# XiYe20/NPVP

Measured on AMD Instinct MI355X. Metric: predictor train frames/sec, higher is better.
Workload: dtype f32 (two-term fp16 split of amax-scaled operands, 3 MFMAs per product, fp32 accumulate: fp32-grade; small GEMMs: three-term bf16 split)

## Files before the change

include/npvp_hip.h:

```cpp
#ifndef NPVP_HIP_H
#define NPVP_HIP_H
#include <stddef.h>
#ifdef __cplusplus
extern "C" {
#endif

typedef struct ihipStream_t* npvp_stream_t;

int npvp_version(void);
const char* npvp_last_error(void);
long long npvp_launch_count(void);
void* npvp_stream_create_low_priority(int* least, int* greatest);
int npvp_stream_destroy(void* stream);
void* npvp_event_create(void);
int npvp_event_record(void* event, void* stream);
float npvp_event_elapsed_ms(void* event0, void* event1);
int npvp_event_destroy(void* event);

long long npvp_graph_node_counts(void* graph, long long* counts, long long* memset_bytes, int max_memsets);

long long npvp_gemm_workspace_bytes(int M, int N, int K);
int npvp_gemm_kernel_id(int a_kc, int b_kc, int M, int N, int K, int precision, int has_planes);
int npvp_gemm_route(int a_kc, int b_kc, int M, int N, int K, int precision, int has_planes, int plain_epilogue, int* out4);
int npvp_gemm_f32(int a_kc, int b_kc, int M, int N, int K, const float* A, long long lda, const float* B, long long ldb,
// ... 15 lines not shown
                              int frames, float eps, npvp_stream_t stream);
int npvp_split_weight(const float* w, long long ld, int N, int K, void* F, void* D, npvp_stream_t stream);
int npvp_split_weights_batched(const void* desc, int count, npvp_stream_t stream);
int npvp_amax(const float* x, long long rows, long long cols, long long ld, float* slot, npvp_stream_t stream);

typedef struct npvp_reduce_job {
  const float* ws; float* out; long long ldc; int M, N, splits, accum; float alpha; int blocks; const float* cs_part; float* cs_out;
} npvp_reduce_job_t;
int npvp_wgrad_f16_chainable(int M, int N, int K);
long long npvp_wgrad_f16_chain_workspace_bytes(int M, int N, int K);
int npvp_wgrad_f16_chained(int M, int N, int K, const float* dy, long long lda, const float* x, long long ldb, float* dw,
                           long long ldc, float* db, int accumulate, const float* a_amax, const float* b_amax,
                           unsigned int* range_flag, float adrop_p, int adrop_g1, int adrop_g2, unsigned int adrop_salt,
                           const unsigned long long* seed, const void* prev_job, void* my_job, void* workspace,
                           long long ws_bytes, npvp_stream_t stream);
int npvp_splitk_reduce_job(const void* job, npvp_stream_t stream);
int npvp_splitk_reduce_multi(const void* jobs, int n, npvp_stream_t stream);
int npvp_linear_bwd_f16_takes(int R, int N, int K);
int npvp_linear_bwd_f16(int R, int N, int K, const float* dy, long long ldy, const float* dy_amax, const void* w_planes_d,
                        const float* w_amax, float* dx, long long ldx, int act, const float* aux_in, const float* residual,
                        long long ldr, float drop_p, int drop_mode, int drop_g1, int drop_g2, unsigned int drop_salt, float* dx_amax,
                        const float* x, long long ldxx, const float* x_amax, float* dw, long long ldw, float* db,
                        unsigned int* range_flag, float adrop_p, int adrop_g1, int adrop_g2, unsigned int adrop_salt,
                        const unsigned long long* seed, const void* prev_job, void* my_job, void* workspace, long long ws_bytes,
                        npvp_stream_t stream);
int npvp_linear_bwd_f16_skip(int R, int N, int K, const float* dy, long long ldy, const float* dy_amax, const void* w_planes_d,
                             const float* w_amax, float* dx, long long ldx, int act, const float* aux_in, const float* residual,
                             long long ldr, float drop_p, int drop_mode, int drop_g1, int drop_g2, unsigned int drop_salt,
                             float* dx_amax, const float* x, long long ldxx, const float* x_amax, float* dw, long long ldw, float* db,
                             unsigned int* range_flag, float adrop_p, int adrop_g1, int adrop_g2, unsigned int adrop_salt,
// ... 220 lines not shown
```

npvp_amd/csrc/gemm.h:

```cpp
#pragma once
#include <type_traits>
#include "common.h"

namespace npvp {

typedef float f32x16 __attribute__((ext_vector_type(16)));
typedef __bf16 bf16x8 __attribute__((ext_vector_type(8)));
typedef __bf16 bf16x4 __attribute__((ext_vector_type(4)));

struct ReduceJob {
  const float* ws; float* out; long long ldc; int M, N, splits, accum; float alpha; int blocks; const float* cs_part; float* cs_out;
};

struct GemmParams {
  const float* A; const float* B; float* C;
  const float* bias;
  const float* residual;
  float* aux_out;
  const float* aux_in;
  float* rowstats;
  float* colsum;
  const unsigned long long* seed;
  long long lda, ldb, ldc, ldr;
  int M, N, K;
// ... 269 lines not shown

inline int wgrad_splits(int M, int N, int K, int min_rows) {
  if ((K & 15) || M < 64 || N < 128 || K < min_rows) return 0;
  const int tiles = ((M + 127) / 128) * ((N + 255) / 256);
  int s = (512 + tiles - 1) / tiles;
  const int maxs = K / 256;
  if (s > maxs) s = maxs;
  if (s > 64) s = 64;
  if (s >= 8) s &= ~7;
  while (s > 1 && (K % (s * 16)) != 0) --s;
  return s < 1 ? 1 : s;
}
inline int wide_wgrad_splits(int M, int N, int K) { return wgrad_splits(M, N, K, 32768); }
inline int f16_wgrad_splits(int M, int N, int K) { return wgrad_splits(M, N, K, 1024); }

inline bool adrop_args_ok(float p, int g1, int g2, const unsigned long long* seed, bool rows16) {
  return p >= 0.f && p < 0.5f && (p == 0.f || (seed && g1 > 0 && g2 > 0 && (!rows16 || g1 % 16 == 0)));
}

int wide_variant(int M, int N, int K);
void launch_gemm_wide(GemmParams& p, int variant, hipStream_t stream);
void launch_gemm_wgrad_wide(GemmParams& p, hipStream_t stream);
int gemm_f16_variant(int M, int N, int K);
void launch_gemm_f16(GemmParams& p, int variant, hipStream_t stream);
void launch_gemm_wgrad_f16(GemmParams& p, hipStream_t stream);

}
```

npvp_amd/csrc/gemm.hip:

```cpp
#include "gemm.h"
#include "partials.h"
#include <type_traits>

namespace npvp {

constexpr int BM = 128, BN = 128, BK = 32, GEMM_THREADS = 256;

template <bool KC> struct Stager;

template <> struct Stager<true> {
  static constexpr int LD = 129;
  float4 r[4];
  __device__ __forceinline__ void load(const float* src, long long ld, int row0, int nrows, int k0) {
    const int t = threadIdx.x;
    const int kc = (t & 7) * 4;
#pragma unroll
    for (int i = 0; i < 4; ++i) {
      const int row = row0 + (t >> 3) + 32 * i;
      r[i] = (row < nrows) ? ld4(src + (long long)row * ld + k0 + kc) : make_float4(0.f, 0.f, 0.f, 0.f);
    }
  }
  __device__ __forceinline__ void store(float* s) const {
    const int t = threadIdx.x;
    const int kc = (t & 7) * 4;
// ... 490 lines not shown
              p.accum, cs_here ? (const float*)p.colsum : nullptr, cs_here ? colsum_a : nullptr, p.c_amax);
  NPVP_CHECK_LAUNCH();
  if (!colsum_a || cs_here) return NPVP_OK;
  return finish_partials(make_partials(p.colsum, 0, p.splits, p.splits, p.M, colsum_a, p.accum).job, 0, stream, "gemm: column-sum reduce launch failed");
}

extern "C" int npvp_gemm_f32_skip(int a_kc, int b_kc, int M, int N, int K, const float* A, long long lda, const float* B,
                                  long long ldb, float* C, long long ldc, const float* bias, int act, const float* aux_in,
                                  float* aux_out, const float* residual, long long ldr, float drop_p, int drop_mode,
                                  int drop_g1, int drop_g2, const unsigned long long* seed, unsigned int salt, float alpha,
                                  int precision, float* colsum_a, const void* b_pre, int accumulate, float* rowstats,
                                  const float* a_amax, const float* b_amax, float* c_amax, unsigned int* range_flag,
                                  float adrop_p, int adrop_g1, int adrop_g2, unsigned int adrop_salt,
                                  float skip_p, int skip_g1, int skip_g2, unsigned int skip_salt,
                                  void* workspace, long long ws_bytes, hipStream_t stream) {
  NPVP_CHECK_ARG(skip_p >= 0.f && skip_p < 1.f && (skip_p == 0.f || (seed && skip_g1 > 0 && skip_g2 > 0 && a_kc)),
                 "gemm: the row skip needs a device seed, row groups and a row-major A");
  NPVP_CHECK_ARG(M > 0 && N > 0 && K > 0, "gemm: empty problem");
  NPVP_CHECK_ARG(precision == 0 || precision == 4 || precision == 5 || precision == 6,
                 "gemm: precision must be 0 (exact fp32-input MFMA), 4 (three-term bf16 split, 6 MFMAs per product: "
                 "fp32-grade), 5 (two-term bf16 split, 3 MFMAs per product, ~2^-16) or 6 (two-term fp16 split with amax-scaled "
                 "operands, 3 MFMAs per product: fp32-grade; shapes it does not take run as 4)");
  const bool want_h = precision == 6;
  NPVP_CHECK_ARG(K % BK == 0, "gemm: K must be a multiple of 32");
  NPVP_CHECK_ARG(M % 4 == 0 && N % 4 == 0, "gemm: M and N must be multiples of 4");
  NPVP_CHECK_ARG(((uintptr_t)A % 16) == 0 && ((uintptr_t)B % 16) == 0 && ((uintptr_t)C % 16) == 0, "gemm: pointers must be 16-byte aligned");
  NPVP_CHECK_ARG(lda % 4 == 0 && ldb % 4 == 0, "gemm: lda/ldb must be multiples of 4 floats");
  NPVP_CHECK_ARG(ldc % 4 == 0 && (!residual || (ldr % 4 == 0 && ((uintptr_t)residual % 16) == 0)) && (!bias || ((uintptr_t)bias % 16) == 0) &&
                 (!aux_in || ((uintptr_t)aux_in % 16) == 0) && (!aux_out || ((uintptr_t)aux_out % 16) == 0),
                 "gemm: ldc / ldr must be multiples of 4 floats and bias / aux / residual 16-byte aligned (float4 epilogue)");
  NPVP_CHECK_ARG(!(a_kc == 0 && b_kc == 1), "gemm: (a_kc=0,b_kc=1) is not used by the path");
  NPVP_CHECK_ARG((act != 3 && act != 4) || aux_in, "gemm: act 3/4 need aux_in");
// ... 75 lines not shown
```

npvp_amd/csrc/gemm_f16.hip:

```cpp
#include "gemm.h"
#include <cstdio>
#include <cstdlib>

namespace npvp {

typedef _Float16 f16x8 __attribute__((ext_vector_type(8)));
typedef _Float16 f16x4 __attribute__((ext_vector_type(4)));
typedef __attribute__((address_space(1))) const void* gptr_t;
typedef __attribute__((address_space(3))) void* lptr_t;
typedef float f32x4 __attribute__((ext_vector_type(4)));

__device__ __forceinline__ void split_f16_scaled(const f32x4 v, const float s, f16x4& hi, f16x4& lo) {
  unsigned int h01, h23, l01, l23;
  asm("v_fma_mixlo_f16 %0, %1, %2, 0" : "=v"(h01) : "v"(v[0]), "v"(s));
  asm("v_fma_mixlo_f16 %0, %1, %2, 0" : "=v"(h23) : "v"(v[2]), "v"(s));
  asm("v_fma_mixhi_f16 %0, %1, %2, 0" : "+v"(h01) : "v"(v[1]), "v"(s));
  asm("v_fma_mixhi_f16 %0, %1, %2, 0" : "+v"(h23) : "v"(v[3]), "v"(s));
  asm("v_fma_mixlo_f16 %0, %1, %2, -%3 op_sel_hi:[0,0,1]" : "=v"(l01) : "v"(v[0]), "v"(s), "v"(h01));
  asm("v_fma_mixlo_f16 %0, %1, %2, -%3 op_sel_hi:[0,0,1]" : "=v"(l23) : "v"(v[2]), "v"(s), "v"(h23));
  asm("v_fma_mixhi_f16 %0, %1, %2, -%3 op_sel:[0,0,1] op_sel_hi:[0,0,1]" : "+v"(l01) : "v"(v[1]), "v"(s), "v"(h01));
  asm("v_fma_mixhi_f16 %0, %1, %2, -%3 op_sel:[0,0,1] op_sel_hi:[0,0,1]" : "+v"(l23) : "v"(v[3]), "v"(s), "v"(h23));
  typedef unsigned int u32x2 __attribute__((ext_vector_type(2)));
  const u32x2 hp = {h01, h23}, lp = {l01, l23};
  hi = __builtin_bit_cast(f16x4, hp);
// ... 301 lines not shown
    float cm = 0.f;
    splitk_reduce_body(p.prev, (by - p.splits) * gx + bx, p.prev.blocks, cm);
    return;
  }
  int z, tl;
  {
    const int tiles = gx;
    if (p.splits > 1 && (p.splits & 7) == 0) {
      const int lin = bx + tiles * by, xcd = lin & 7, slot = lin >> 3;
      const int g = slot / tiles;
      tl = slot - g * tiles; z = g * 8 + xcd;
    } else { z = by; tl = bx; }
  }
  const int tile_m = tl / p.tiles_n, tile_n = tl - tile_m * p.tiles_n;
  const int m0 = tile_m * BM, n0 = tile_n * BN;
  const float* A = p.A + (long long)z * p.K * p.lda;
  const float* B = p.B + (long long)z * p.K * p.ldb;
  const int t = threadIdx.x, lane = t & 63, wave = __builtin_amdgcn_readfirstlane(t >> 6);
  const int wm = wave / WN, wn = wave % WN, r = lane & 31, h = lane >> 5;
  const int nk = p.K >> 4;
  const float sa = amax_scale(amax_slot_read(p.a_amax)), sb = amax_scale(amax_slot_read(p.b_amax));

  f32x16 acc[TM][TN];
#pragma unroll
  for (int i = 0; i < TM; ++i)
#pragma unroll
    for (int j = 0; j < TN; ++j)
#pragma unroll
      for (int g = 0; g < 16; ++g) acc[i][j][g] = 0.f;

  const int ka = t >> 5, cqa = t & 31, kb = t >> 6, cqb = t & 63;
  const char* a_base = reinterpret_cast<const char*>(A);
  const char* b_base = reinterpret_cast<const char*>(B);
  const unsigned int a_voff = (unsigned int)(((long long)ka * p.lda + min(m0 + 4 * cqa, p.M - 4)) * 4);
  const unsigned int b_voff = (unsigned int)(((long long)kb * p.ldb + min(n0 + 4 * cqb, p.N - 4)) * 4);
  const long long a_row8 = 32 * p.lda, b_row4 = 16 * p.ldb, a_step = 64 * p.lda, b_step = 64 * p.ldb;
  const int a_dst = ka * ROWA + ((8 * cqa) ^ ((ka & 3) << 6));
  const int b_dst = A_BYTES + kb * ROWB + ((8 * cqb) ^ ((kb & 3) << 6));
  const int q = (lane >> 2) & 3, pp = lane & 3, cg = 16 * ((lane >> 4) & 1) + 4 * pp;
  int fa[TM], fb[TN];
#pragma unroll
  for (int i = 0; i < TM; ++i) fa[i] = (8 * h + q) * ROWA + (((wm * TM * 32 + i * 32 + cg) * 2) ^ (q << 6));
#pragma unroll
  for (int j = 0; j < TN; ++j) fb[j] = A_BYTES + (8 * h + q) * ROWB + (((wn * TN * 32 + j * 32 + cg) * 2) ^ (q << 6));

  const bool want_cs = p.colsum && tile_n == 0;
  f32x4 cs = {0.f, 0.f, 0.f, 0.f};
  f32x4 cm4 = {0.f, 0.f, 0.f, 0.f};
  f32x4 ra[2], rb[4];
#define NPVP_G_LOAD(KT)                                                                                     \
  { const int kt_ = min((KT), nk - 1);                                                                      \
    const char* pa_ = a_base + (long long)kt_ * a_step; const char* pb_ = b_base + (long long)kt_ * b_step;  \
    asm volatile("global_load_dwordx4 %0, %1, %2" : "=v"(ra[0]) : "v"(a_voff), "s"(pa_) : "memory");        \
    asm volatile("global_load_dwordx4 %0, %1, %2" : "=v"(ra[1]) : "v"(a_voff), "s"(pa_ + a_row8) : "memory"); \
    _Pragma("unroll") for (int i_ = 0; i_ < 4; ++i_)                                                        \
      asm volatile("global_load_dwordx4 %0, %1, %2" : "=v"(rb[i_]) : "v"(b_voff), "s"(pb_ + i_ * b_row4) : "memory"); }
#define NPVP_G_WAIT(N, ...) asm volatile("s_waitcnt vmcnt(" #N ")" : __VA_ARGS__ :: "memory");
#define NPVP_G_STORE(DST, V, SC, PLANE)                                                                     \
  { f16x4 hi_, lo_; split_f16_scaled((V), (SC), hi_, lo_);                                                  \
    *reinterpret_cast<f16x4*>(DST) = hi_; *reinterpret_cast<f16x4*>((DST) + (PLANE)) = lo_; }
  const unsigned long long aseed = p.adrop.thresh ? *p.seed : 0ull;
  const long long arow0 = (long long)z * p.K;
  float am_ = 1.f;
#define NPVP_G_AMASK(KT) { if (p.adrop.thresh) am_ = drop_spec_scale(p.adrop, aseed, arow0 + 16ll * min((KT), nk - 1), 0, 1); }
#define NPVP_G_STORE_A(ST) { const float sam_ = sa * am_;                                                                        \
    if (p.range_flag) cm4 = __builtin_elementwise_max(cm4, __builtin_elementwise_max(__builtin_elementwise_abs(ra[0]), __builtin_elementwise_abs(ra[1]))); \
    NPVP_G_STORE((ST) + a_dst, ra[0], sam_, A_PLANE) NPVP_G_STORE((ST) + a_dst + 8 * ROWA, ra[1], sam_, A_PLANE) }
#define NPVP_G_STORE_B(ST, I) NPVP_G_STORE((ST) + b_dst + (I) * 4 * ROWB, rb[I], sb, B_PLANE)

  NPVP_G_LOAD(0)
  NPVP_G_AMASK(0)
  NPVP_G_WAIT(0, "+v"(ra[0]), "+v"(ra[1]), "+v"(rb[0]), "+v"(rb[1]), "+v"(rb[2]), "+v"(rb[3]))
  if (want_cs) cs += (ra[0] + ra[1]) * am_;
  NPVP_G_STORE_A(lds)
  NPVP_G_STORE_B(lds, 0) NPVP_G_STORE_B(lds, 1) NPVP_G_STORE_B(lds, 2) NPVP_G_STORE_B(lds, 3)
  NPVP_G_LOAD(1)
  __syncthreads();

#define NPVP_G_STEP(KT, CUR, NXT)                                                                            \
  {                                                                                                          \
    const char* st_ = lds + (CUR) * STAGE;                                                                   \
    char* nx_ = lds + (NXT) * STAGE;                                                                         \
    NPVP_G_WAIT(3, "+v"(ra[0]), "+v"(ra[1]), "+v"(rb[0]))                                                    \
    NPVP_G_AMASK((KT) + 1)                                                         \
    if (want_cs && (KT) + 1 < nk) { asm volatile("" ::: "memory"); cs += (ra[0] + ra[1]) * am_; }   \
    f16x8 fa_[TM][2];                                                                                        \
    _Pragma("unroll") for (int i_ = 0; i_ < TM; ++i_)                                                        \
      _Pragma("unroll") for (int s_ = 0; s_ < 2; ++s_) fa_[i_][s_] = lds_read_tr_pair_h(st_ + fa[i_] + s_ * A_PLANE, 4 * ROWA); \
// ... 9 lines not shown
    }                                                                                                        \
     \
    __builtin_amdgcn_sched_barrier(0);                                                                       \
    asm volatile("s_waitcnt lgkmcnt(0)" ::: "memory");                                                       \
    __builtin_amdgcn_s_barrier();                                                                            \
  }

  int kt = 0;
  for (; kt + 1 < nk; kt += 2) {
    NPVP_G_STEP(kt, 0, 1)
    NPVP_G_STEP(kt + 1, 1, 0)
  }
  if (kt < nk) NPVP_G_STEP(kt, 0, 1)
  asm volatile("s_waitcnt vmcnt(0)" : "+v"(ra[0]), "+v"(ra[1]), "+v"(rb[0]), "+v"(rb[1]), "+v"(rb[2]), "+v"(rb[3]) :: "memory");
  if (p.range_flag) {
    float* red = reinterpret_cast<float*>(lds);
    *reinterpret_cast<f32x4*>(red + ka * BM + 4 * cqa) = cm4;
    __syncthreads();
    bool flag = false;
    if (t < BM) {
      float m = red[t];
#pragma unroll
      for (int i = 1; i < 8; ++i) m = fmaxf(m, red[i * BM + t]);
      const int et = (int)((__float_as_uint(sa) >> 23) & 0xffu), e = (int)((__float_as_uint(m) >> 23) & 0xffu);
      const int d = 268 - et - e;
      flag = e >= 16 && e != 255 && d >= 18 && m0 + t < p.M;
    }
    const bool any = __builtin_amdgcn_ballot_w64(flag) != 0ull;
    if (any && lane == 0) atomicAdd(p.range_flag, 1u);
    __syncthreads();
// ... 68 lines not shown
  long long want = (total4 + 255) / 256;
  if (want > 256) want = 256;
  if (want < 1) want = 1;
  return (int)((want + tiles - 1) / tiles);
}

static dim3 size_gemm_wgrad_f16(GemmParams& p) {
  p.tiles_m = (p.M + 127) / 128;
  p.tiles_n = (p.N + 255) / 256;
  const int tiles = p.tiles_m * p.tiles_n, rr = reduce_rows_for(p.prev, tiles);
  p.prev.blocks = rr * tiles;
  return dim3(tiles, p.splits + rr);
}

void launch_gemm_wgrad_f16(GemmParams& p, hipStream_t stream) {
  const dim3 grid = size_gemm_wgrad_f16(p);
  NPVP_LAUNCH((gemm_wgrad_f16_kernel<2, 4, 2, 2>), grid, dim3(256), 0, stream, p);
}

static bool deferred_wgrad_args_ok(const char* who, const float* dy, long long lda, const float* x, long long ldb, const float* dw, long long ldc, float adrop_p,
                                   int adrop_g1, int adrop_g2, const unsigned long long* seed, const void* workspace, long long ws_bytes, long long ws_need) {
  const char* what = ((((uintptr_t)dy | (uintptr_t)x | (uintptr_t)dw) & 15) || ((lda | ldb | ldc) & 3)) ? "operands must be 16-byte aligned with leading dimensions that are multiples of 4"
                     : !adrop_args_ok(adrop_p, adrop_g1, adrop_g2, seed, true) ? "adrop needs a device seed and groups of a multiple of 16 rows"
                     : (!workspace || ws_bytes < ws_need) ? "workspace too small" : nullptr;
  char msg[192];
  if (what) { snprintf(msg, sizeof(msg), "%s: %s", who, what); npvp_set_error(msg); }
  return !what;
}

static GemmParams deferred_wgrad_params(int M, int N, int K, const float* dy, long long lda, const float* x, long long ldb, const float* a_amax, const float* b_amax,
// ... 157 lines not shown
  NPVP_CHECK_LAUNCH();
  return NPVP_OK;
}

static_assert(sizeof(ReduceJob) == sizeof(npvp_reduce_job_t), "npvp_reduce_job_t (include/npvp_hip.h) mirrors this layout");

extern "C" int npvp_wgrad_f16_chainable(int M, int N, int K) {
  return (M % 4 == 0 && N % 4 == 0 && f16_wgrad_splits(M, N, K) > 1) ? 1 : 0;
}

extern "C" long long npvp_wgrad_f16_chain_workspace_bytes(int M, int N, int K) {
  const int s = f16_wgrad_splits(M, N, K);
  return s > 1 ? splitk_workspace_bytes(s, M, N) : 0;
}

extern "C" int npvp_wgrad_f16_chained(int M, int N, int K, const float* dy, long long lda, const float* x, long long ldb, float* dw,
                                      long long ldc, float* db, int accumulate, const float* a_amax, const float* b_amax,
                                      unsigned int* range_flag, float adrop_p, int adrop_g1, int adrop_g2, unsigned int adrop_salt,
                                      const unsigned long long* seed, const void* prev_job, void* my_job, void* workspace,
                                      long long ws_bytes, hipStream_t stream) {
  NPVP_CHECK_ARG(npvp_wgrad_f16_chainable(M, N, K), "wgrad_f16_chained: shape not taken (npvp_wgrad_f16_chainable tells)");
  NPVP_CHECK_ARG(dy && x && dw && a_amax && b_amax && my_job, "wgrad_f16_chained: null operand / amax slot / job");
  if (!deferred_wgrad_args_ok("wgrad_f16_chained", dy, lda, x, ldb, dw, ldc, adrop_p, adrop_g1, adrop_g2, seed, workspace, ws_bytes,
                              npvp_wgrad_f16_chain_workspace_bytes(M, N, K))) return NPVP_ERR_ARG;
  NPVP_CHECK_ARG(!db || ((uintptr_t)db % 16) == 0, "wgrad_f16_chained: the bias gradient must be 16-byte aligned");
  GemmParams p = deferred_wgrad_params(M, N, K, dy, lda, x, ldb, a_amax, b_amax, range_flag, make_drop_spec(adrop_p, adrop_salt, 1, adrop_g1, adrop_g2),
                                       seed, prev_job, workspace, db != nullptr, accumulate);
  launch_gemm_wgrad_f16(p, stream);
  NPVP_CHECK_LAUNCH();
  leave_reduce_job(p, dw, ldc, db, my_job);
  return NPVP_OK;
}

extern "C" int npvp_linear_bwd_f16_takes(int R, int N, int K) {
  const int v = gemm_f16_variant(R, K, N);
  return ((v == 2 || v == 3 || v == 4) && npvp_wgrad_f16_chainable(N, K, R)) ? 1 : 0;
}

extern "C" int npvp_linear_bwd_f16_skip(int R, int N, int K, const float* dy, long long ldy, const float* dy_amax, const void* w_planes_d,
                                        const float* w_amax, float* dx, long long ldx, int act, const float* aux_in, const float* residual,
                                        long long ldr, float drop_p, int drop_mode, int drop_g1, int drop_g2, unsigned int drop_salt,
                                        float* dx_amax, const float* x, long long ldxx, const float* x_amax, float* dw, long long ldw, float* db,
                                        unsigned int* range_flag, float adrop_p, int adrop_g1, int adrop_g2, unsigned int adrop_salt,
                                        float skip_p, int skip_g1, int skip_g2, unsigned int skip_salt,
                                        const unsigned long long* seed, const void* prev_job, void* my_job, void* workspace,
                                        long long ws_bytes, hipStream_t stream) {
// ... 98 lines not shown
```

npvp_amd/ops.py:

```python
import functools
import os
from collections import namedtuple

import torch

from ._lib import lib, check
from . import sched as _S
from .sched import (_p, _ptr, _stream, _ws, AmaxSlot, GemmProbe, HbmProbe, ProbeEvent, AuxStream, StepContext, current, use, scoped,
                    remember, rng, GradSink, WgradStream, WgradChain, ReduceQueue, RangeGuard)


def amax_of(t, slot=None):
    if slot is not None:
        return slot
    for cand in (t, t._base):
        tag = getattr(cand, "_npvp_amax", None) if cand is not None else None
        if tag is not None and tag[1] == cand._version:
            return tag[0]
    s = AmaxSlot.new(t.device)
    t2 = t if t.dim() == 2 else t.reshape(-1, t.shape[-1])
    if t2.stride(1) != 1:
        t2 = t2.contiguous()
    check(lib().npvp_amax(_ptr(t2), t2.shape[0], t2.shape[1], t2.stride(0), _ptr(s), _stream()), "npvp_amax")
    t._npvp_amax = (s, t._version)
# ... 358 lines not shown

def masked_grad(dy2, drop, w):
    if not drop.on:
        return dy2, NO_DROP
    R, N = dy2.shape
    K = w.shape[1]
    if (drop.mode == 1 and drop.g1 % 16 == 0 and drop.p < 0.5 and GEMM_PRECISION == 6 and R <= DROP_PATH_IN_GEMM_ROWS
            and _planes(w, "D", R) is not None and _gemm_kernel_id(1, 0, R, K, N, 6, True) in (5, 7) and _h16(N, K, R, 6)):
        return dy2, drop
    return drop_apply(dy2, drop), NO_DROP


DROP_PATH_IN_GEMM_ROWS = 1 << 30


def linear_wgrad(dy, x, with_bias_grad=False, into=None, into_b=None, dy_amax=None, x_amax=None, a_drop=NO_DROP):
    R, N = dy.shape
    K = x.shape[1]
    acc = into is not None
    dw = into if acc else torch.empty(N, K, dtype=torch.float32, device=dy.device)
    db = (into_b if acc else torch.empty(N, dtype=torch.float32, device=dy.device)) if with_bias_grad else None
    c = _S._cur
    g = c.range_guard
    plan = wgrad_plan(N, K, R, GEMM_PRECISION, WGRAD_PRECISION, acc, a_drop.on, g.fallback, g.strict, c.wgrad.in_flush, c.wgrad.enabled,
                      c.grad_sink.listener is not None, c.chain.enabled, dy.stride(1) == 1 and x.stride(1) == 1 and dw.stride(1) == 1)
    flag = g.flag(dy.device) if plan.watch else None
    if plan.route == "strict":
        tw = torch.empty(N, K, dtype=torch.float32, device=dy.device)
        tb = torch.empty(N, dtype=torch.float32, device=dy.device) if with_bias_grad else None
        gemm(0, 0, N, K, R, dy, dy.stride(0), x, x.stride(0), tw, colsum_a=tb, a_amax=dy_amax, b_amax=x_amax, range_flag=flag)
        if g.poll(dy.device):
            g.fallback = False
            gemm(0, 0, N, K, R, dy, dy.stride(0), x, x.stride(0), tw, colsum_a=tb, precision=4)
        if acc:
            dw.add_(tw)
            if tb is not None:
                db.add_(tb)
        else:
            dw, db = tw, tb
    elif plan.route == "chained":
        c.chain.launch(dy, x, dw, db, amax_of(dy, dy_amax), amax_of(x, x_amax), a_drop, flag)
    else:
        gemm(0, 0, N, K, R, dy, dy.stride(0), x, x.stride(0), dw, colsum_a=db, accumulate=acc, precision=plan.precision, a_amax=dy_amax,
             b_amax=x_amax, a_drop=a_drop, range_flag=flag)
    return (dw, db) if with_bias_grad else dw


class FusedLinearBwd:
    enabled = True
    MAX_ROWS = 16384
    with_gradient_stream = False

    @classmethod
    def takes(cls, R, N, K):
        return linear_bwd_plan(R, N, K, 6, True, False, True, True, True, True, False, cls.MAX_ROWS).fused


def linear_bwd(dy, x, w, b, sk, act=0, aux_in=None, drop=NO_DROP, residual=None, dy_amax=None, dx_amax=None, a_drop=NO_DROP,
               row_skip=NO_DROP):
    R, N = dy.shape
    K = w.shape[1]
    has_b = b is not None
    c = _S._cur
    sunk = _sunk(sk, has_b)
    pl = _planes(w, "D", R)
    plan = linear_bwd_plan(R, N, K, GEMM_PRECISION, sunk, c.wgrad.enabled, not (c.range_guard.fallback or c.range_guard.strict),
                           dy.stride(1) == 1 and x.stride(1) == 1 and (not sunk or sk[0][0].stride(1) == 1), pl is not None,
                           FusedLinearBwd.enabled, FusedLinearBwd.with_gradient_stream, FusedLinearBwd.MAX_ROWS)
    if not plan.fused:
        dx = linear_dgrad(dy, w, act=act, aux_in=aux_in, drop=drop, residual=residual, dy_amax=dy_amax, dx_amax=dx_amax, a_drop=a_drop,
                          row_skip=row_skip)
        gw, gb = _lin_grads(dy, x, w, b, sk, a_drop=a_drop, plan=plan)
        return dx, gw, gb
    planes, w_amax = pl
    gw, gb = sk[0][0], (sk[1][0] if has_b else None)
    dev = dy.device
    dy_amax, x_amax = amax_of(dy, dy_amax), amax_of(x)
    dx = torch.empty(R, K, dtype=torch.float32, device=dev)
    ws, wsn = _ws(c.chain.workspace_bytes(N, K, R), dev)
    st = _stream()
    seed = c.rng.seed_tensor(dev) if (drop.on or a_drop.on or row_skip.on) else None
    outs = (gw.data_ptr(),) if gb is None else (gw.data_ptr(), gb.data_ptr())
    later = c.chain if plan.reduction == "chained" else c.reduce
    job_addr, prev_addr = later.job_slot(st, outs)
    pe = GemmProbe.begin(8)
    head = (R, N, K, dy.data_ptr(), dy.stride(0), dy_amax.data_ptr(), planes.data_ptr(), w_amax.data_ptr(), dx.data_ptr(), dx.stride(0),
            act, _ptr(aux_in), _ptr(residual), 0 if residual is None else residual.stride(0), drop.p, drop.mode, drop.g1, drop.g2,
# ... 418 lines not shown
        if ctx.needs_input_grad[0] and ctx.needs_input_grad[1]:
            dz, ad = masked_grad(dy2, ctx.drop, w)
        else:
            dz, ad = (drop_apply(dy2, ctx.drop) if ctx.drop.on else dy2), NO_DROP
        dx = linear_dgrad(dz, w, a_drop=ad).reshape(ctx.xshape) if ctx.needs_input_grad[0] else None
        dw = db = None
        want_b = ctx.has_b and ctx.needs_input_grad[2]
        if ctx.needs_input_grad[1]:
            dw, db = _lin_grads(dz, x2, w, True if want_b else None, ctx.sink, a_drop=ad)
        elif want_b:
            db = colsum(dz)
        dres = dy if ctx.has_r else None
        return dx, dw, db, dres, None, None


def _lin_grads(dy, x, w, b, sk, a_drop=NO_DROP, plan=None):
    has_b = b is not None
    if plan is None:
        plan = linear_bwd_plan(dy.shape[0], dy.shape[1], x.shape[1], GEMM_PRECISION, _sunk(sk, has_b), _S._cur.wgrad.enabled)
    if not plan.sunk:
        g = linear_wgrad(dy, x, has_b, a_drop=a_drop)
        return (g[0], g[1]) if has_b else (g, None)
    a1, a2 = (amax_of(dy), amax_of(x)) if plan.fill_slots else (None, None)
    fn = lambda dy=dy, x=x, gw=sk[0][0], gb=(sk[1][0] if has_b else None), a1=a1, a2=a2, ad=a_drop: \
        linear_wgrad(dy, x, has_b, into=gw, into_b=gb, dy_amax=a1, x_amax=a2, a_drop=ad)
    if plan.on_grad_stream:
        _S._cur.wgrad.run(fn, dy, x, wrote=sk, urgent=plan.urgent)
    else:
        fn()
        _S._cur.grad_sink.wrote(*sk)
    return None, None


def _wb_sink(w, b):
    sw = _S._cur.grad_sink.slot(w)
    if sw is None:
        return None
    if b is None or not b.requires_grad:
        return (sw, None)
    sb = _S._cur.grad_sink.slot(b)
# ... 450 lines not shown
            gdww = gdwb = None
        else:
            gdww = torch.empty(hid, 1, 3, 3, dtype=torch.float32, device=dev)
            check(L.npvp_transpose(_ptr(dwtb), _ptr(gdww), 1, 9, hid, _stream()), "npvp_transpose")
            gdwb = dwtb[9]
        dh1, gn1w, gn1b = _fln_bwd(da1, h1, stats[0], stats[1], n1w, n1b, frames, 64 * hid, NO_DROP, NO_DROP, 1, s_n1,
                                      psum=psum, nparts=nparts, skip=skip)
        del da1
        dx, gw1, gb1 = linear_bwd(dh1, x, w1, True if has_b1 else None, s_fc1, row_skip=rs)
        return (dx, dout if has_res else None, gw1, gb1, gn1w, gn1b, gdww, gdwb, gn2w, gn2b, gw2, gb2, gn3w, gn3b,
                None, None, None, None)


MID_BWD_N2 = True
DROP_PATH_SKIP = True


def mlpdwbn_fused_supported(R, C, hid, Co, H, W):
    return (GEMM_PRECISION in (4, 6) and H == 8 and W == 8 and R % 64 == 0 and hid % 512 == 0 and Co % 128 == 0 and hid % 128 == 0
            and C % 32 == 0)


def mlpdwbn(x, res, w1, b1, n1w, n1b, dww, dwb, n2w, n2b, w2, b2, n3w, n3b, frames, T, p_drop, p_dp):
    return _MlpDwbn.apply(x, res, w1, b1, n1w, n1b, dww, dwb, n2w, n2b, w2, b2, n3w, n3b, frames, T, p_drop, p_dp)


def _raw_ln_fwd(x2, w, b, eps, relu=0):
    rows, C = x2.shape
    y = torch.empty_like(x2)
    st = torch.empty(2, rows, dtype=torch.float32, device=x2.device)
# ... 658 lines not shown
```

npvp_amd/sched.py:

```python
import contextlib
import ctypes
import functools
import os

import torch

from ._lib import lib, check

_p = ctypes.c_void_p


def _ptr(t):
    return None if t is None else t.data_ptr()


_raw_stream = getattr(torch._C, "_cuda_getCurrentRawStream", None)
_cur_dev = getattr(torch._C, "_cuda_getDevice", None) or torch.cuda.current_device


def _stream():
    if _raw_stream is not None:
        return _raw_stream(_cur_dev())
    return torch.cuda.current_stream().cuda_stream

# ... 447 lines not shown

    def job_added(self, st, out_ptrs, keep, wrote):
        job, prev = self._open
        if prev is not None and prev[2] is not None:
            self.ctx.grad_sink.wrote(*prev[2])
        self._pending[st] = (job, keep, wrote)
        if not self.ctx.wgrad.in_flush:
            self.ctx.reduce.arm()

    def launch(self, dy, x, dw, db, dy_amax, x_amax, a_drop, flag):
        R, N = dy.shape
        K = x.shape[1]
        st = _stream()
        ws, wsn = _ws(self.workspace_bytes(N, K, R), dy.device)
        job_addr, prev_addr = self.job_slot(st)
        seed = self.ctx.rng.seed_tensor(dy.device) if a_drop.on else None
        pe = GemmProbe.begin(6)
        check(lib().npvp_wgrad_f16_chained(N, K, R, _ptr(dy), dy.stride(0), _ptr(x), x.stride(0), _ptr(dw), dw.stride(0), _ptr(db), 1,
                                           _ptr(dy_amax), _ptr(x_amax), _ptr(flag), a_drop.p, a_drop.g1, a_drop.g2, a_drop.salt,
                                           _ptr(seed), prev_addr, job_addr, _ptr(ws), wsn, st), "npvp_wgrad_f16_chained")
        GemmProbe.end(pe, 2.0 * N * K * R, 4.0 * (N * R + K * R + N * K), (0, 0), 6)
        self.job_added(st, None, (ws, dw, db), None)

    def flush(self):
        st = _stream()
        prev = self._pending.pop(st, None)
        if prev is not None:
            check(lib().npvp_splitk_reduce_job(ctypes.addressof(prev[0]), st), "npvp_splitk_reduce_job")
            if prev[2] is not None:
                self.ctx.grad_sink.wrote(*prev[2])


class RangeGuardState:
    mode = os.environ.get("NPVP_RANGE_GUARD", "on")
    strict = mode == "strict"
# ... 146 lines not shown
```

Before: 8443.

## Skip dropped drop-path row groups in the chained fp16 weight-gradient GEMM

The split-K fp16 weight-gradient kernel now builds, per block, a compacted list of row groups (K-dimension instances) kept by the drop-path mask. It then iterates only over their K steps, redistributing the remaining steps evenly across splits. The mask is evaluated with a ballot and prefix count in shared memory. Python routes the row-skip spec into the chained and generic wgrad paths. This avoids loading and multiplying rows whose gradient is zero because the whole sample path was dropped. The cost is extra per-block setup, a readfirstlane-indexed address walk, and handling of splits that end up empty.

```diff
diff --git a/include/npvp_hip.h b/include/npvp_hip.h
--- a/include/npvp_hip.h
+++ b/include/npvp_hip.h
@@ -53,6 +53,11 @@
                            unsigned int* range_flag, float adrop_p, int adrop_g1, int adrop_g2, unsigned int adrop_salt,
                            const unsigned long long* seed, const void* prev_job, void* my_job, void* workspace,
                            long long ws_bytes, npvp_stream_t stream);
+int npvp_wgrad_f16_chained_skip(int M, int N, int K, const float* dy, long long lda, const float* x, long long ldb, float* dw,
+                                long long ldc, float* db, int accumulate, const float* a_amax, const float* b_amax,
+                                unsigned int* range_flag, float adrop_p, int adrop_g1, int adrop_g2, unsigned int adrop_salt,
+                                float skip_p, int skip_g1, int skip_g2, unsigned int skip_salt, const unsigned long long* seed,
+                                const void* prev_job, void* my_job, void* workspace, long long ws_bytes, npvp_stream_t stream);
 int npvp_splitk_reduce_job(const void* job, npvp_stream_t stream);
 int npvp_splitk_reduce_multi(const void* jobs, int n, npvp_stream_t stream);
 int npvp_linear_bwd_f16_takes(int R, int N, int K);
diff --git a/npvp_amd/csrc/gemm.h b/npvp_amd/csrc/gemm.h
--- a/npvp_amd/csrc/gemm.h
+++ b/npvp_amd/csrc/gemm.h
@@ -307,6 +307,16 @@
 inline int wide_wgrad_splits(int M, int N, int K) { return wgrad_splits(M, N, K, 32768); }
 inline int f16_wgrad_splits(int M, int N, int K) { return wgrad_splits(M, N, K, 1024); }
 
+constexpr int KSKIP_MAX_INSTANCES = 256;
+__host__ __device__ inline int kskip_real_step(const unsigned short* kept, int S, int j) { return (int)kept[j / S] * S + j % S; }
+__host__ __device__ inline void kskip_split_range(int nkk, int splits, int z, int& j0, int& j1) {
+  const long long q = ((long long)nkk + splits - 1) / splits, a = q * z, b = a + q;
+  j0 = (int)(a < nkk ? a : nkk); j1 = (int)(b < nkk ? b : nkk);
+}
+inline bool kskip_takes(long long rows, int g1) {
+  return g1 > 0 && g1 % 16 == 0 && rows % g1 == 0 && rows / g1 <= KSKIP_MAX_INSTANCES;
+}
+
 inline bool adrop_args_ok(float p, int g1, int g2, const unsigned long long* seed, bool rows16) {
   return p >= 0.f && p < 0.5f && (p == 0.f || (seed && g1 > 0 && g2 > 0 && (!rows16 || g1 % 16 == 0)));
 }
diff --git a/npvp_amd/csrc/gemm.hip b/npvp_amd/csrc/gemm.hip
--- a/npvp_amd/csrc/gemm.hip
+++ b/npvp_amd/csrc/gemm.hip
@@ -528,8 +528,8 @@
                                   float adrop_p, int adrop_g1, int adrop_g2, unsigned int adrop_salt,
                                   float skip_p, int skip_g1, int skip_g2, unsigned int skip_salt,
                                   void* workspace, long long ws_bytes, hipStream_t stream) {
-  NPVP_CHECK_ARG(skip_p >= 0.f && skip_p < 1.f && (skip_p == 0.f || (seed && skip_g1 > 0 && skip_g2 > 0 && a_kc)),
-                 "gemm: the row skip needs a device seed, row groups and a row-major A");
+  NPVP_CHECK_ARG(skip_p >= 0.f && skip_p < 1.f && (skip_p == 0.f || (seed && skip_g1 > 0 && skip_g2 > 0 && (a_kc || !b_kc))),
+                 "gemm: the row skip needs a device seed, row groups and a row-major A or a weight-gradient layout");
   NPVP_CHECK_ARG(M > 0 && N > 0 && K > 0, "gemm: empty problem");
   NPVP_CHECK_ARG(precision == 0 || precision == 4 || precision == 5 || precision == 6,
                  "gemm: precision must be 0 (exact fp32-input MFMA), 4 (three-term bf16 split, 6 MFMAs per product: "
diff --git a/npvp_amd/csrc/gemm_f16.hip b/npvp_amd/csrc/gemm_f16.hip
--- a/npvp_amd/csrc/gemm_f16.hip
+++ b/npvp_amd/csrc/gemm_f16.hip
@@ -339,11 +339,34 @@
   }
   const int tile_m = tl / p.tiles_n, tile_n = tl - tile_m * p.tiles_n;
   const int m0 = tile_m * BM, n0 = tile_n * BN;
-  const float* A = p.A + (long long)z * p.K * p.lda;
-  const float* B = p.B + (long long)z * p.K * p.ldb;
   const int t = threadIdx.x, lane = t & 63, wave = __builtin_amdgcn_readfirstlane(t >> 6);
   const int wm = wave / WN, wn = wave % WN, r = lane & 31, h = lane >> 5;
-  const int nk = p.K >> 4;
+  __shared__ unsigned short kept_inst[KSKIP_MAX_INSTANCES];
+  __shared__ int kept_wave[NW];
+  int nk = p.K >> 4, kstep0 = z * nk;
+  int S = 0x7fffffff, wstep = 0, winst = 0;
+  if (p.rskip.thresh) {
+    const int I = (int)((long long)p.K * p.splits / p.rskip.g1);
+    const unsigned int grp = (unsigned int)t - div_by_magic((unsigned int)t, p.rskip.m2, p.rskip.s2) * (unsigned int)p.rskip.g2;
+    const bool keep = t < I && rng_u32(*p.seed, p.rskip.salt, (uint64_t)grp) >= p.rskip.thresh;
+    const unsigned long long bal = __builtin_amdgcn_ballot_w64(keep);
+    if (lane == 0) kept_wave[wave] = __builtin_popcountll(bal);
+    __syncthreads();
+    int before = 0, kept = 0;
+#pragma unroll
+    for (int w = 0; w < NW; ++w) { const int c = kept_wave[w]; before += w < wave ? c : 0; kept += c; }
+    if (keep) kept_inst[before + __builtin_popcountll(bal & ((1ull << lane) - 1ull))] = (unsigned short)t;
+    __syncthreads();
+    kept = __builtin_amdgcn_readfirstlane(kept);
+    S = p.rskip.g1 >> 4;
+    int j0, j1;
+    kskip_split_range(S * kept, p.splits, z, j0, j1);
+    nk = j1 - j0; kstep0 = 0;
+    if (nk > 0) {
+      winst = j0 / S; wstep = j0 - winst * S;
+      kstep0 = __builtin_amdgcn_readfirstlane((int)kept_inst[winst]) * S + wstep;
+    }
+  }
   const float sa = amax_scale(amax_slot_read(p.a_amax)), sb = amax_scale(amax_slot_read(p.b_amax));
 
   f32x16 acc[TM][TN];
@@ -355,8 +378,8 @@
       for (int g = 0; g < 16; ++g) acc[i][j][g] = 0.f;
 
   const int ka = t >> 5, cqa = t & 31, kb = t >> 6, cqb = t & 63;
-  const char* a_base = reinterpret_cast<const char*>(A);
-  const char* b_base = reinterpret_cast<const char*>(B);
+  const char* a_base = reinterpret_cast<const char*>(p.A);
+  const char* b_base = reinterpret_cast<const char*>(p.B);
   const unsigned int a_voff = (unsigned int)(((long long)ka * p.lda + min(m0 + 4 * cqa, p.M - 4)) * 4);
   const unsigned int b_voff = (unsigned int)(((long long)kb * p.ldb + min(n0 + 4 * cqb, p.N - 4)) * 4);
   const long long a_row8 = 32 * p.lda, b_row4 = 16 * p.ldb, a_step = 64 * p.lda, b_step = 64 * p.ldb;
@@ -373,9 +396,13 @@
   f32x4 cs = {0.f, 0.f, 0.f, 0.f};
   f32x4 cm4 = {0.f, 0.f, 0.f, 0.f};
   f32x4 ra[2], rb[4];
+  int kld = kstep0;
 #define NPVP_G_LOAD(KT)                                                                                     \
-  { const int kt_ = min((KT), nk - 1);                                                                      \
-    const char* pa_ = a_base + (long long)kt_ * a_step; const char* pb_ = b_base + (long long)kt_ * b_step;  \
+  { if ((KT) > 0 && (KT) < nk) {                                                                            \
+      ++kld;                                                                                                \
+      if (++wstep == S) { wstep = 0; ++winst; kld = __builtin_amdgcn_readfirstlane((int)kept_inst[winst]) * S; } \
+    }                                                                                                       \
+    const char* pa_ = a_base + (long long)kld * a_step; const char* pb_ = b_base + (long long)kld * b_step;  \
     asm volatile("global_load_dwordx4 %0, %1, %2" : "=v"(ra[0]) : "v"(a_voff), "s"(pa_) : "memory");        \
     asm volatile("global_load_dwordx4 %0, %1, %2" : "=v"(ra[1]) : "v"(a_voff), "s"(pa_ + a_row8) : "memory"); \
     _Pragma("unroll") for (int i_ = 0; i_ < 4; ++i_)                                                        \
@@ -385,9 +412,8 @@
   { f16x4 hi_, lo_; split_f16_scaled((V), (SC), hi_, lo_);                                                  \
     *reinterpret_cast<f16x4*>(DST) = hi_; *reinterpret_cast<f16x4*>((DST) + (PLANE)) = lo_; }
   const unsigned long long aseed = p.adrop.thresh ? *p.seed : 0ull;
-  const long long arow0 = (long long)z * p.K;
   float am_ = 1.f;
-#define NPVP_G_AMASK(KT) { if (p.adrop.thresh) am_ = drop_spec_scale(p.adrop, aseed, arow0 + 16ll * min((KT), nk - 1), 0, 1); }
+#define NPVP_G_AMASK(KT) { if (p.adrop.thresh) am_ = drop_spec_scale(p.adrop, aseed, 16ll * kld, 0, 1); }
 #define NPVP_G_STORE_A(ST) { const float sam_ = sa * am_;                                                                        \
     if (p.range_flag) cm4 = __builtin_elementwise_max(cm4, __builtin_elementwise_max(__builtin_elementwise_abs(ra[0]), __builtin_elementwise_abs(ra[1]))); \
     NPVP_G_STORE((ST) + a_dst, ra[0], sam_, A_PLANE) NPVP_G_STORE((ST) + a_dst + 8 * ROWA, ra[1], sam_, A_PLANE) }
@@ -396,7 +422,7 @@
   NPVP_G_LOAD(0)
   NPVP_G_AMASK(0)
   NPVP_G_WAIT(0, "+v"(ra[0]), "+v"(ra[1]), "+v"(rb[0]), "+v"(rb[1]), "+v"(rb[2]), "+v"(rb[3]))
-  if (want_cs) cs += (ra[0] + ra[1]) * am_;
+  if (want_cs && nk > 0) cs += (ra[0] + ra[1]) * am_;
   NPVP_G_STORE_A(lds)
   NPVP_G_STORE_B(lds, 0) NPVP_G_STORE_B(lds, 1) NPVP_G_STORE_B(lds, 2) NPVP_G_STORE_B(lds, 3)
   NPVP_G_LOAD(1)
@@ -436,6 +462,7 @@
   if (kt < nk) NPVP_G_STEP(kt, 0, 1)
   asm volatile("s_waitcnt vmcnt(0)" : "+v"(ra[0]), "+v"(ra[1]), "+v"(rb[0]), "+v"(rb[1]), "+v"(rb[2]), "+v"(rb[3]) :: "memory");
   if (p.range_flag) {
+    if (nk == 0) cm4 = f32x4{0.f, 0.f, 0.f, 0.f};
     float* red = reinterpret_cast<float*>(lds);
     *reinterpret_cast<f32x4*>(red + ka * BM + 4 * cqa) = cm4;
     __syncthreads();
@@ -534,6 +561,7 @@
 }
 
 void launch_gemm_wgrad_f16(GemmParams& p, hipStream_t stream) {
+  if (p.rskip.thresh && !(p.seed && kskip_takes((long long)p.K * p.splits, p.rskip.g1))) p.rskip.thresh = 0u;
   const dim3 grid = size_gemm_wgrad_f16(p);
   NPVP_LAUNCH((gemm_wgrad_f16_kernel<2, 4, 2, 2>), grid, dim3(256), 0, stream, p);
 }
@@ -721,11 +749,14 @@
   return s > 1 ? splitk_workspace_bytes(s, M, N) : 0;
 }
 
-extern "C" int npvp_wgrad_f16_chained(int M, int N, int K, const float* dy, long long lda, const float* x, long long ldb, float* dw,
-                                      long long ldc, float* db, int accumulate, const float* a_amax, const float* b_amax,
-                                      unsigned int* range_flag, float adrop_p, int adrop_g1, int adrop_g2, unsigned int adrop_salt,
-                                      const unsigned long long* seed, const void* prev_job, void* my_job, void* workspace,
-                                      long long ws_bytes, hipStream_t stream) {
+extern "C" int npvp_wgrad_f16_chained_skip(int M, int N, int K, const float* dy, long long lda, const float* x, long long ldb, float* dw,
+                                           long long ldc, float* db, int accumulate, const float* a_amax, const float* b_amax,
+                                           unsigned int* range_flag, float adrop_p, int adrop_g1, int adrop_g2, unsigned int adrop_salt,
+                                           float skip_p, int skip_g1, int skip_g2, unsigned int skip_salt,
+                                           const unsigned long long* seed, const void* prev_job, void* my_job, void* workspace,
+                                           long long ws_bytes, hipStream_t stream) {
+  NPVP_CHECK_ARG(skip_p >= 0.f && skip_p < 1.f && (skip_p == 0.f || (seed && skip_g1 > 0 && skip_g2 > 0)),
+                 "wgrad_f16_chained: the row skip needs a device seed and row groups");
   NPVP_CHECK_ARG(npvp_wgrad_f16_chainable(M, N, K), "wgrad_f16_chained: shape not taken (npvp_wgrad_f16_chainable tells)");
   NPVP_CHECK_ARG(dy && x && dw && a_amax && b_amax && my_job, "wgrad_f16_chained: null operand / amax slot / job");
   if (!deferred_wgrad_args_ok("wgrad_f16_chained", dy, lda, x, ldb, dw, ldc, adrop_p, adrop_g1, adrop_g2, seed, workspace, ws_bytes,
@@ -733,10 +764,20 @@
   NPVP_CHECK_ARG(!db || ((uintptr_t)db % 16) == 0, "wgrad_f16_chained: the bias gradient must be 16-byte aligned");
   GemmParams p = deferred_wgrad_params(M, N, K, dy, lda, x, ldb, a_amax, b_amax, range_flag, make_drop_spec(adrop_p, adrop_salt, 1, adrop_g1, adrop_g2),
                                        seed, prev_job, workspace, db != nullptr, accumulate);
+  p.rskip = make_drop_spec(skip_p, skip_salt, 1, skip_g1, skip_g2);
   launch_gemm_wgrad_f16(p, stream);
   NPVP_CHECK_LAUNCH();
   leave_reduce_job(p, dw, ldc, db, my_job);
   return NPVP_OK;
+}
+
+extern "C" int npvp_wgrad_f16_chained(int M, int N, int K, const float* dy, long long lda, const float* x, long long ldb, float* dw,
+                                      long long ldc, float* db, int accumulate, const float* a_amax, const float* b_amax,
+                                      unsigned int* range_flag, float adrop_p, int adrop_g1, int adrop_g2, unsigned int adrop_salt,
+                                      const unsigned long long* seed, const void* prev_job, void* my_job, void* workspace,
+                                      long long ws_bytes, hipStream_t stream) {
+  return npvp_wgrad_f16_chained_skip(M, N, K, dy, lda, x, ldb, dw, ldc, db, accumulate, a_amax, b_amax, range_flag, adrop_p, adrop_g1,
+                                     adrop_g2, adrop_salt, 0.f, 1, 1, 0u, seed, prev_job, my_job, workspace, ws_bytes, stream);
 }
 
 extern "C" int npvp_linear_bwd_f16_takes(int R, int N, int K) {
diff --git a/npvp_amd/ops.py b/npvp_amd/ops.py
--- a/npvp_amd/ops.py
+++ b/npvp_amd/ops.py
@@ -396,7 +396,16 @@
 DROP_PATH_IN_GEMM_ROWS = 1 << 30
 
 
-def linear_wgrad(dy, x, with_bias_grad=False, into=None, into_b=None, dy_amax=None, x_amax=None, a_drop=NO_DROP):
+class _MaskAndSkip:
+    __slots__ = ("on", "p", "g1", "g2", "salt", "row_skip")
+
+    def __init__(self, a_drop, row_skip):
+        self.on, self.p, self.g1, self.g2, self.salt, self.row_skip = a_drop.on, a_drop.p, a_drop.g1, a_drop.g2, a_drop.salt, row_skip
+
+
+def linear_wgrad(dy, x, with_bias_grad=False, into=None, into_b=None, dy_amax=None, x_amax=None, a_drop=NO_DROP, row_skip=NO_DROP):
+    if not WGRAD_K_SKIP:
+        row_skip = NO_DROP
     R, N = dy.shape
     K = x.shape[1]
     acc = into is not None
@@ -421,10 +430,11 @@
         else:
             dw, db = tw, tb
     elif plan.route == "chained":
-        c.chain.launch(dy, x, dw, db, amax_of(dy, dy_amax), amax_of(x, x_amax), a_drop, flag)
+        c.chain.launch(dy, x, dw, db, amax_of(dy, dy_amax), amax_of(x, x_amax), _MaskAndSkip(a_drop, row_skip) if row_skip.on else a_drop,
+                       flag)
     else:
         gemm(0, 0, N, K, R, dy, dy.stride(0), x, x.stride(0), dw, colsum_a=db, accumulate=acc, precision=plan.precision, a_amax=dy_amax,
-             b_amax=x_amax, a_drop=a_drop, range_flag=flag)
+             b_amax=x_amax, a_drop=a_drop, range_flag=flag, row_skip=row_skip)
     return (dw, db) if with_bias_grad else dw
 
 
@@ -452,7 +462,7 @@
     if not plan.fused:
         dx = linear_dgrad(dy, w, act=act, aux_in=aux_in, drop=drop, residual=residual, dy_amax=dy_amax, dx_amax=dx_amax, a_drop=a_drop,
                           row_skip=row_skip)
-        gw, gb = _lin_grads(dy, x, w, b, sk, a_drop=a_drop, plan=plan)
+        gw, gb = _lin_grads(dy, x, w, b, sk, a_drop=a_drop, plan=plan, row_skip=NO_DROP if FusedLinearBwd.takes(R, N, K) else row_skip)
         return dx, gw, gb
     planes, w_amax = pl
     gw, gb = sk[0][0], (sk[1][0] if has_b else None)
@@ -901,16 +911,16 @@
         return dx, dw, db, dres, None, None
 
 
-def _lin_grads(dy, x, w, b, sk, a_drop=NO_DROP, plan=None):
+def _lin_grads(dy, x, w, b, sk, a_drop=NO_DROP, plan=None, row_skip=NO_DROP):
     has_b = b is not None
     if plan is None:
         plan = linear_bwd_plan(dy.shape[0], dy.shape[1], x.shape[1], GEMM_PRECISION, _sunk(sk, has_b), _S._cur.wgrad.enabled)
     if not plan.sunk:
-        g = linear_wgrad(dy, x, has_b, a_drop=a_drop)
+        g = linear_wgrad(dy, x, has_b, a_drop=a_drop, row_skip=row_skip)
         return (g[0], g[1]) if has_b else (g, None)
     a1, a2 = (amax_of(dy), amax_of(x)) if plan.fill_slots else (None, None)
-    fn = lambda dy=dy, x=x, gw=sk[0][0], gb=(sk[1][0] if has_b else None), a1=a1, a2=a2, ad=a_drop: \
-        linear_wgrad(dy, x, has_b, into=gw, into_b=gb, dy_amax=a1, x_amax=a2, a_drop=ad)
+    fn = lambda dy=dy, x=x, gw=sk[0][0], gb=(sk[1][0] if has_b else None), a1=a1, a2=a2, ad=a_drop, rs=row_skip: \
+        linear_wgrad(dy, x, has_b, into=gw, into_b=gb, dy_amax=a1, x_amax=a2, a_drop=ad, row_skip=rs)
     if plan.on_grad_stream:
         _S._cur.wgrad.run(fn, dy, x, wrote=sk, urgent=plan.urgent)
     else:
@@ -1391,6 +1401,7 @@
 
 MID_BWD_N2 = True
 DROP_PATH_SKIP = True
+WGRAD_K_SKIP = True
 
 
 def mlpdwbn_fused_supported(R, C, hid, Co, H, W):
diff --git a/npvp_amd/sched.py b/npvp_amd/sched.py
--- a/npvp_amd/sched.py
+++ b/npvp_amd/sched.py
@@ -485,11 +485,16 @@
         st = _stream()
         ws, wsn = _ws(self.workspace_bytes(N, K, R), dy.device)
         job_addr, prev_addr = self.job_slot(st)
-        seed = self.ctx.rng.seed_tensor(dy.device) if a_drop.on else None
+        rs = getattr(a_drop, "row_skip", None)
+        seed = self.ctx.rng.seed_tensor(dy.device) if (a_drop.on or rs is not None) else None
         pe = GemmProbe.begin(6)
-        check(lib().npvp_wgrad_f16_chained(N, K, R, _ptr(dy), dy.stride(0), _ptr(x), x.stride(0), _ptr(dw), dw.stride(0), _ptr(db), 1,
-                                           _ptr(dy_amax), _ptr(x_amax), _ptr(flag), a_drop.p, a_drop.g1, a_drop.g2, a_drop.salt,
-                                           _ptr(seed), prev_addr, job_addr, _ptr(ws), wsn, st), "npvp_wgrad_f16_chained")
+        head = (N, K, R, _ptr(dy), dy.stride(0), _ptr(x), x.stride(0), _ptr(dw), dw.stride(0), _ptr(db), 1, _ptr(dy_amax), _ptr(x_amax),
+                _ptr(flag), a_drop.p, a_drop.g1, a_drop.g2, a_drop.salt)
+        tail = (_ptr(seed), prev_addr, job_addr, _ptr(ws), wsn, st)
+        if rs is not None:
+            check(lib().npvp_wgrad_f16_chained_skip(*head, rs.p, rs.g1, rs.g2, rs.salt, *tail), "npvp_wgrad_f16_chained_skip")
+        else:
+            check(lib().npvp_wgrad_f16_chained(*head, *tail), "npvp_wgrad_f16_chained")
         GemmProbe.end(pe, 2.0 * N * K * R, 4.0 * (N * R + K * R + N * K), (0, 0), 6)
         self.job_added(st, None, (ws, dw, db), None)
 
```

New measurement: 8487, median of 6. Within noise of the previous version (+0.5%).
